# wuer5/OMGSR

Hardware: AMD Instinct MI355X
Metric: SR images/sec (higher is better)
Workload: dtype fp16; 1 GPU; OMGSR-S 256->1024, batch=4/GPU, accurate tier (fp32 stream, fp16 MFMA operands + split corrections), tiled VAE 256/64; global_batch=4, latent_tile=64, tile_overlap=32, world_size=1, parallelism=dp1, weights=seeded random, SD2.1-base shapes

## Files before the change

include/omgsr_hip.h:

```cpp
#ifndef OMGSR_HIP_H
#define OMGSR_HIP_H

#include <stdint.h>

#ifdef __cplusplus
extern "C" {
#endif

#define OMGSR_E_BADARG (-1)
#define OMGSR_E_SHAPE (-2)
#define OMGSR_E_ARCH (-3)

#define OMGSR_ACT_NONE 0
#define OMGSR_ACT_SILU 1
#define OMGSR_ACT_GELU_TANH 2
#define OMGSR_ACT_GEGLU 3

#define OMGSR_OUT_BF16 0
#define OMGSR_OUT_F32 1

#define OMGSR_LAYOUT_NHWC 0
#define OMGSR_LAYOUT_T 1

#define OMGSR_EL_16 0
// ... 108 lines not shown
                                 int32_t G, int32_t act, int32_t stat_rows, int32_t x_el, int32_t y_el, void* y2, int32_t y2_el,
                                 uint32_t* overflow_flag, void* stream);
typedef struct omgsr_gn_apply_group {
    const void* x;
    void* y;
    void* y2;
    int64_t HW;
    int32_t rows;
    int32_t reserved;
} omgsr_gn_apply_group;
int omgsr_groupnorm_apply_multi(const omgsr_gn_apply_group* groups, int32_t ngroups, const float* mean, const float* rstd,
                                const float* gamma, const float* beta, int32_t C, int32_t G, int32_t act, int32_t stat_rows,
                                int32_t x_el, int32_t y_el, int32_t y2_el, uint32_t* overflow_flag, void* stream);
int omgsr_groupnorm_apply_mxfp8(const void* x, void* codes, void* scales, const float* mean, const float* rstd, const float* gamma,
                                const float* beta, int32_t rows, int64_t HW, int32_t C, int32_t G, int32_t act, int32_t stat_rows,
                                int32_t x_el, void* stream);
int omgsr_groupnorm_apply_mxfp8_c64(const void* x, void* codes, void* scales, const float* mean, const float* rstd, const float* gamma,
                                    const float* beta, int32_t rows, int64_t HW, int32_t C, int32_t G, int32_t act, int32_t stat_rows,
                                    int32_t x_el, void* stream);
int omgsr_groupnorm_apply_mxfp8_multi(const omgsr_gn_apply_group* groups, int32_t ngroups, const float* mean, const float* rstd,
                                      const float* gamma, const float* beta, int32_t C, int32_t G, int32_t act, int32_t stat_rows,
                                      int32_t x_el, void* stream);
typedef struct omgsr_edge_group {
    const void* x;
    void* y;
    int32_t rows;
    int32_t H;
    int32_t W;
    int32_t reserved;
} omgsr_edge_group;
int omgsr_conv_out_gn(const omgsr_edge_group* groups, int32_t ngroups, const float* mean, const float* rstd, const float* gamma,
                      const float* beta, const float* weight, const float* bias, int32_t Cin, int32_t Cout, int32_t G, int32_t stat_rows,
                      void* stream);
int omgsr_groupnorm_finalize2(const float* partial_a, int32_t nslot_a, int32_t Ca, const float* partial_b, int32_t nslot_b, int32_t Cb,
                              float* mean, float* rstd, float* var_out, int32_t N, int32_t G, double count, float eps, void* stream);
int omgsr_groupnorm_apply2(const void* xa, const void* xb, int32_t Ca, void* y, const float* mean, const float* rstd, const float* gamma,
                           const float* beta, int32_t N, int64_t HW, int32_t C, int32_t G, int32_t act, int32_t y_el, void* y2, int32_t y2_el,
                           uint32_t* overflow_flag, void* stream);

int omgsr_layernorm(const void* x, void* y, const float* a, const float* b, int64_t rows, int32_t C,
                    float eps, int32_t x_el, int32_t y_el, void* stream);
int omgsr_quantize_mxfp8(const void* x, int32_t x_el, int64_t rows, int32_t K, int64_t x_ld, void* codes, void* scales, void* stream);
int omgsr_quantize_mxfp8_ld(const void* x, int32_t x_el, int64_t rows, int32_t K, int64_t x_ld, void* codes, void* scales, int64_t c_ld,
                            int64_t s_ld, void* stream);
int omgsr_layernorm_mxfp8(const void* x, const float* a, const float* b, int64_t rows, int32_t C, float eps, int32_t x_el, void* codes,
                          void* scales, int64_t c_ld, int64_t s_ld, void* stream);
int omgsr_to_operand(const float* x, void* y, int64_t rows, int32_t C, int32_t y_el, uint32_t* overflow_flag, void* stream);
int omgsr_transpose_split(const float* x, void* y, int32_t B, int32_t L, int32_t C, int64_t ld, void* stream);

typedef struct omgsr_attn_args {
    const void* q; const void* k; const void* vt; void* o;
    int32_t B, H, D, Lq, Lk;
    int64_t q_ld, k_ld, vt_ld, o_ld;
    int64_t q_bstride, k_bstride, vt_bstride, o_bstride;
    float scale;
    int32_t o_lo_off;
    int32_t o_mx;
    int32_t q_lo_off;
    int32_t k_lo_off;
    int32_t p_split;
    int32_t reserved1;
    int64_t vt_lo_off;
    int32_t qkv_el;
    int32_t qkv_reserved;
    const uint8_t* q_scale;
    const uint8_t* k_scale;
// ... 67 lines not shown
```

omgsr_amd/_lib.py:

```python
from __future__ import annotations

import ctypes as C
import os

import torch

from .build import lib_path

ABI_VERSION = 22


class OmgsrError(RuntimeError):
    pass


class IgemmArgs(C.Structure):
    _fields_ = [
        ("in_", C.c_void_p), ("weight", C.c_void_p), ("bias", C.c_void_p), ("gate", C.c_void_p),
        ("residual", C.c_void_p), ("out", C.c_void_p),
        ("N", C.c_int32), ("H", C.c_int32), ("W", C.c_int32), ("Cin", C.c_int32),
        ("Cout", C.c_int32), ("Cout_pad", C.c_int32), ("K_pad", C.c_int32),
        ("R", C.c_int32), ("S", C.c_int32), ("stride", C.c_int32), ("pad_top", C.c_int32),
        ("pad_left", C.c_int32), ("upsample", C.c_int32),
        ("Ho", C.c_int32), ("Wo", C.c_int32),
        ("act", C.c_int32), ("out_dtype", C.c_int32), ("out_layout", C.c_int32),
        ("t_rows", C.c_int32), ("t_ld", C.c_int32), ("out_ld", C.c_int32),
        ("batch", C.c_int32),
        ("in_bstride", C.c_int64), ("w_bstride", C.c_int64), ("out_bstride", C.c_int64),
        ("alpha", C.c_float), ("weight_cm", C.c_void_p), ("workspace", C.c_void_p),
        ("gn_partial", C.c_void_p), ("gn_groups", C.c_int32), ("gn_entries", C.c_int32),
        ("res_el", C.c_int32), ("in_split", C.c_int32), ("sample_rows", C.c_int64), ("out_lo_off", C.c_int32),
        ("in_ld", C.c_int32), ("w_split", C.c_int32), ("weight_ph", C.c_void_p), ("mx_chunks16", C.c_int32), ("mx_scale_w1", C.c_int32), ("mx_scale_a1", C.c_int32),
        ("mx_scale_w2", C.c_int32), ("mx_scale_a2", C.c_int32), ("out_mx", C.c_int32), ("group_tiles", C.c_int32), ("overflow_flag", C.c_void_p),
        ("gn_scale_shift", C.c_void_p), ("gn_nimg", C.c_int32), ("gn_act", C.c_int32), ("in_el", C.c_int32), ("mx_fmt", C.c_int32),
        ("mxf8", C.c_int32), ("mxf8_reserved", C.c_int32), ("in_scale", C.c_void_p), ("w_scale", C.c_void_p),
    ]


GN_MAX_GROUPS = 8


class GnMergeArgs(C.Structure):
    _fields_ = [("partial", C.c_void_p * GN_MAX_GROUPS), ("count", C.c_double * GN_MAX_GROUPS),
                ("weight", C.c_float * GN_MAX_GROUPS), ("tiles", C.c_int32 * GN_MAX_GROUPS),
                ("nslot", C.c_int32 * GN_MAX_GROUPS), ("entries", C.c_int32 * GN_MAX_GROUPS), ("ngroups", C.c_int32)]


class GnApplyGroup(C.Structure):
    _fields_ = [("x", C.c_void_p), ("y", C.c_void_p), ("y2", C.c_void_p), ("HW", C.c_int64), ("rows", C.c_int32), ("reserved", C.c_int32)]


class EdgeGroup(C.Structure):
    _fields_ = [("x", C.c_void_p), ("y", C.c_void_p), ("rows", C.c_int32), ("H", C.c_int32), ("W", C.c_int32), ("reserved", C.c_int32)]


class AttnArgs(C.Structure):
    _fields_ = [
        ("q", C.c_void_p), ("k", C.c_void_p), ("vt", C.c_void_p), ("o", C.c_void_p),
        ("B", C.c_int32), ("H", C.c_int32), ("D", C.c_int32), ("Lq", C.c_int32), ("Lk", C.c_int32),
        ("q_ld", C.c_int64), ("k_ld", C.c_int64), ("vt_ld", C.c_int64), ("o_ld", C.c_int64),
        ("q_bstride", C.c_int64), ("k_bstride", C.c_int64), ("vt_bstride", C.c_int64), ("o_bstride", C.c_int64),
        ("scale", C.c_float), ("o_lo_off", C.c_int32), ("o_mx", C.c_int32), ("q_lo_off", C.c_int32), ("k_lo_off", C.c_int32), ("p_split", C.c_int32),
        ("reserved1", C.c_int32), ("vt_lo_off", C.c_int64),
        ("qkv_el", C.c_int32), ("qkv_reserved", C.c_int32), ("q_scale", C.c_void_p), ("k_scale", C.c_void_p), ("vt_scale", C.c_void_p),
        ("q_sld", C.c_int64), ("k_sld", C.c_int64), ("vt_sld", C.c_int64), ("q_sbstride", C.c_int64), ("k_sbstride", C.c_int64),
        ("vt_sbstride", C.c_int64),
    ]


class TimingEntry(C.Structure):
    _fields_ = [("kind", C.c_int32), ("ms", C.c_float), ("flops", C.c_double), ("bytes", C.c_double),
                ("m", C.c_int64), ("n", C.c_int64), ("k", C.c_int64), ("variant", C.c_int32), ("stage", C.c_int32)]


_P, _I, _L, _F = C.c_void_p, C.c_int32, C.c_int64, C.c_float

SIGNATURES = {
    "omgsr_abi_version": (C.c_int, []),
    "omgsr_check_device": (C.c_int, []),
    "omgsr_set_compute_dtype": (C.c_int, [C.c_int]),
    "omgsr_get_compute_dtype": (C.c_int, []),
    "omgsr_error_string": (C.c_char_p, [C.c_int]),
    "omgsr_igemm": (C.c_int, [C.POINTER(IgemmArgs), _P]),
    "omgsr_igemm_out_mxfp8": (C.c_int, [C.POINTER(IgemmArgs), _P, _L, _P]),
    "omgsr_igemm_mxfp8_multi_ok": (C.c_int32, [C.POINTER(IgemmArgs), _I]),
    "omgsr_igemm_mxfp8_multi": (C.c_int, [C.POINTER(IgemmArgs), _I, _P]),
    "omgsr_igemm_multi_plan": (C.c_int, [C.POINTER(IgemmArgs), _I]),
    "omgsr_igemm_multi": (C.c_int, [C.POINTER(IgemmArgs), _I, _P]),
    "omgsr_set_batch_invariant": (C.c_int, [C.c_int]),
    "omgsr_set_attention_defer_max": (C.c_int, [C.c_float]),
    "omgsr_igemm_workspace_bytes": (C.c_int64, [C.POINTER(IgemmArgs)]),
    "omgsr_igemm_gn_slots": (C.c_int32, [C.POINTER(IgemmArgs)]),
    "omgsr_igemm_gn_entries": (C.c_int32, [C.POINTER(IgemmArgs)]),
    "omgsr_igemm_gn_fusable": (C.c_int32, [C.POINTER(IgemmArgs)]),
    "omgsr_igemm_out_mx6_ok": (C.c_int32, [C.POINTER(IgemmArgs)]),
    "omgsr_conv_mxfp8_ok": (C.c_int32, [C.POINTER(IgemmArgs)]),
    "omgsr_conv_mxfp8": (C.c_int, [C.POINTER(IgemmArgs), _P]),
    "omgsr_conv_mxfp8_multi_ok": (C.c_int32, [C.POINTER(IgemmArgs), _I]),
    "omgsr_conv_mxfp8_multi": (C.c_int, [C.POINTER(IgemmArgs), _I, _P]),
    "omgsr_conv_mxfp8_up_ok": (C.c_int32, [C.POINTER(IgemmArgs)]),
    "omgsr_conv_mxfp8_up": (C.c_int, [C.POINTER(IgemmArgs), _P]),
    "omgsr_conv_mxfp8_up_multi_ok": (C.c_int32, [C.POINTER(IgemmArgs), _I]),
    "omgsr_conv_mxfp8_up_multi": (C.c_int, [C.POINTER(IgemmArgs), _I, _P]),
    "omgsr_conv_mxfp8_deep_ok": (C.c_int32, [C.POINTER(IgemmArgs)]),
    "omgsr_conv_mxfp8_deep": (C.c_int, [C.POINTER(IgemmArgs), _P]),
    "omgsr_groupnorm_apply_mxfp8": (C.c_int, [_P, _P, _P, _P, _P, _P, _P, _I, _L, _I, _I, _I, _I, _I, _P]),
    "omgsr_groupnorm_apply_mxfp8_c64": (C.c_int, [_P, _P, _P, _P, _P, _P, _P, _I, _L, _I, _I, _I, _I, _I, _P]),
    "omgsr_groupnorm_apply_mxfp8_multi": (C.c_int, [C.POINTER(GnApplyGroup), _I, _P, _P, _P, _P, _I, _I, _I, _I, _I, _P]),
    "omgsr_groupnorm_scale_shift": (C.c_int, [_P, _P, _P, _P, _P, _I, _I, _I, _P]),
    "omgsr_groupnorm_finalize": (C.c_int, [_P, _P, _P, _P, _I, _I, _I, _I, C.c_double, _F, _P]),
    "omgsr_groupnorm_partial": (C.c_int, [_P, _P, _I, _L, _I, _I, _I, _P]),
    "omgsr_groupnorm_finalize_merged": (C.c_int, [C.POINTER(GnMergeArgs), _P, _P, _P, _I, _I, _F, _P]),
    "omgsr_groupnorm_apply_shared": (C.c_int, [_P, _P, _P, _P, _P, _P, _I, _L, _I, _I, _I, _I, _I, _I, _P, _I, _P, _P]),
    "omgsr_groupnorm_apply_multi": (C.c_int, [C.POINTER(GnApplyGroup), _I, _P, _P, _P, _P, _I, _I, _I, _I, _I, _I, _I, _P, _P]),
    "omgsr_conv_out_gn": (C.c_int, [C.POINTER(EdgeGroup), _I, _P, _P, _P, _P, _P, _P, _I, _I, _I, _I, _P]),
    "omgsr_groupnorm_finalize2": (C.c_int, [_P, _I, _I, _P, _I, _I, _P, _P, _P, _I, _I, C.c_double, _F, _P]),
    "omgsr_groupnorm_apply2": (C.c_int, [_P, _P, _I, _P, _P, _P, _P, _P, _I, _L, _I, _I, _I, _I, _P, _I, _P, _P]),
    "omgsr_image_to_model_input": (C.c_int, [_P, _P, _I, _I, _I, _I, _P]),
    "omgsr_colorfix_workspace_bytes": (C.c_int64, [_I, _I, _I, _I]),
    "omgsr_colorfix": (C.c_int, [_P, _I, _P, _P, _P, _I, _I, _I, _I, _I, _P]),
    "omgsr_groupnorm_nchunk": (C.c_int, [_L]),
    "omgsr_groupnorm_stats": (C.c_int, [_P, _P, _P, _P, _P, _I, _L, _I, _I, _F, _I, _P]),
    "omgsr_groupnorm_apply": (C.c_int, [_P, _P, _P, _P, _P, _P, _I, _L, _I, _I, _I, _I, _I, _P, _I, _P, _P]),
    "omgsr_layernorm": (C.c_int, [_P, _P, _P, _P, _L, _I, _F, _I, _I, _P]),
    "omgsr_resize_nearest_exact_nhwc": (C.c_int, [_P, _P, _I, _I, _I, _I, _I, _I, _F, _F, _I, _P]),
    "omgsr_transpose_split": (C.c_int, [_P, _P, _I, _I, _I, _L, _P]),
    "omgsr_to_operand": (C.c_int, [_P, _P, _L, _I, _I, _P, _P]),
    "omgsr_quantize_mxfp8": (C.c_int, [_P, _I, _L, _I, _L, _P, _P, _P]),
    "omgsr_quantize_mxfp8_ld": (C.c_int, [_P, _I, _L, _I, _L, _P, _P, _L, _L, _P]),
    "omgsr_layernorm_mxfp8": (C.c_int, [_P, _P, _P, _L, _I, _F, _I, _P, _P, _L, _L, _P]),
    "omgsr_attention": (C.c_int, [C.POINTER(AttnArgs), _P]),
    "omgsr_softmax_rows": (C.c_int, [_P, _P, _L, _I, _I, _P]),
    "omgsr_softmax_rows_split": (C.c_int, [_P, _P, _L, _I, _I, _P]),
    "omgsr_rmsnorm_rope": (C.c_int, [_P, _P, _P, _I, _P, _P, _I, _I, _I, _I, _L, _I, _I, _F, _P]),
    "omgsr_rmsnorm_rope_mxfp8": (C.c_int, [_P, _P, _P, _I, _P, _P, _I, _I, _I, _I, _L, _I, _I, _F, _P, _P, _L, _L, _P]),
    "omgsr_nchw_to_nhwc": (C.c_int, [_P, _P, _I, _I, _I, _I, _I, _I, _I, _P]),
    "omgsr_nhwc_to_nchw": (C.c_int, [_P, _P, _I, _I, _I, _I, _I, _I, _I, _F, _F, _I, _P]),
    "omgsr_copy_channels": (C.c_int, [_P, _P, _L, _I, _I, _I, _I, _I, _P]),
    "omgsr_vae_sample": (C.c_int, [_P, _P, _P, _L, _I, _I, _F, _F, _I, _P]),
    "omgsr_axpby": (C.c_int, [_P, _P, _P, _L, _F, _F, _F, _F, _I, _I, _P]),
    "omgsr_linear_f32": (C.c_int, [_P, _P, _P, _P, _I, _I, _I, _I, _P]),
    "omgsr_tile_accumulate": (C.c_int, [_P, _P, _P, _I, _I, _I, _I, _I, _I, _I, _I, _I, _I, _P]),
    "omgsr_tile_normalise": (C.c_int, [_P, _P, _P, _I, _L, _I, _I, _I, _P]),
    "omgsr_crop_nhwc": (C.c_int, [_P, _P, _I, _I, _I, _I, _I, _I, _I, _I, _I, _P]),
    "omgsr_paste_nhwc": (C.c_int, [_P, _P] + [_I] * 13 + [_P]),
    "omgsr_flux_pack": (C.c_int, [_P, _P, _I, _I, _I, _I, _I, _I, _I, _P]),
    "omgsr_resample_u8": (C.c_int, [_P, _P, _P, _P, _I, _I, _I, _I, _I, _I, _P]),
    "omgsr_timing_enable": (C.c_int, [C.c_int]),
# ... 37 lines not shown
```

omgsr_amd/build.py:

```python
from __future__ import annotations

import hashlib
import os
import shutil
import subprocess
import sys

HERE = os.path.dirname(os.path.abspath(__file__))
CSRC = os.path.join(HERE, "csrc")
LIBDIR = os.path.join(HERE, "lib")
LIBNAME = "libomgsr_hip.so"
SOURCES = ["igemm.hip", "igemm_dma.hip", "igemm_p8.hip", "igemm_gmx.hip", "igemm_halo.hip", "igemm_halo_f16.hip", "igemm_halo_multi.hip", "igemm_halo_mx.hip", "igemm_halo_mx6.hip", "igemm_halo_mx6_flat.hip", "igemm_halo_out6.hip", "igemm_halo_flat.hip", "igemm_halo_gn.hip", "attention.hip", "norm.hip", "elementwise.hip", "colorfix.hip", "preprocess.hip", "mfma_peak.hip", "gemm_mxfp8.hip", "gemm_mxfp8_out8.hip", "gemm_mxfp8_multi.hip", "attention_mxfp8.hip", "attention_d512.hip", "conv_mxfp8.hip", "conv_mxfp8_up.hip", "conv_mxfp8_deep.hip", "conv_edge.hip"]
ARCH = "gfx950"


def lib_path() -> str:
    return os.path.join(LIBDIR, LIBNAME)


def _source_digest() -> str:
    h = hashlib.sha256()
    names = sorted(os.listdir(CSRC)) + [os.path.join("..", "..", "include", "omgsr_hip.h")]
    for n in names:
        p = os.path.join(CSRC, n)
        if os.path.isfile(p):
            h.update(n.encode())
            with open(p, "rb") as f:
                h.update(f.read())
    return h.hexdigest()


def build_library(force: bool = False, verbose: bool = False) -> str:
    hipcc = shutil.which("hipcc") or "/opt/rocm/bin/hipcc"
    os.makedirs(LIBDIR, exist_ok=True)
    out = lib_path()
    stamp = out + ".sha256"
    defs = ["-DOMGSR_BUILD_ABLATIONS"] if os.environ.get("OMGSR_BUILD_ABLATIONS", "0") == "1" else []
    defs += os.environ.get("OMGSR_EXTRA_DEFS", "").split()
    digest = _source_digest() + "".join(defs)
    if not force and os.path.isfile(out) and os.path.isfile(stamp) and open(stamp).read().strip() == digest:
        return out
    if not os.path.exists(hipcc):
        raise RuntimeError("hipcc not found: cannot build libomgsr_hip.so")
    from concurrent.futures import ThreadPoolExecutor

# ... 117 lines not shown
```

omgsr_amd/diffusers_api/autoencoder_kl.py:

```python
from __future__ import annotations

import os
from types import SimpleNamespace
from typing import Optional

import torch
import torch.nn as nn

from .. import ops
from ..nn import Conv2d, GroupNorm, Linear, norm_silu_conv
from .modeling_utils import ConfigDict, ModelMixin

SD21_VAE_CONFIG = dict(in_channels=3, out_channels=3, block_out_channels=[128, 256, 512, 512], layers_per_block=2,
                       latent_channels=4, norm_num_groups=32, scaling_factor=0.18215, shift_factor=None,
                       use_quant_conv=True, use_post_quant_conv=True, act_fn="silu", sample_size=768)
FLUX_VAE_CONFIG = dict(in_channels=3, out_channels=3, block_out_channels=[128, 256, 512, 512], layers_per_block=2,
                       latent_channels=16, norm_num_groups=32, scaling_factor=0.3611, shift_factor=0.1159,
                       use_quant_conv=False, use_post_quant_conv=False, act_fn="silu", sample_size=1024)


class ResnetBlock2D(nn.Module):
    def __init__(self, in_channels: int, out_channels: int, temb_channels: Optional[int], groups: int, eps: float):
        super().__init__()
        self.in_channels, self.out_channels = in_channels, out_channels
        self.norm1 = GroupNorm(groups, in_channels, eps=eps)
        self.conv1 = Conv2d(in_channels, out_channels, 3, padding=1)
        self.time_emb_proj = Linear(temb_channels, out_channels) if temb_channels else None
        self.norm2 = GroupNorm(groups, out_channels, eps=eps)
        self.conv2 = Conv2d(out_channels, out_channels, 3, padding=1)
        self.use_in_shortcut = in_channels != out_channels
        self.conv_shortcut = Conv2d(in_channels, out_channels, 1) if self.use_in_shortcut else None
        self.nonlinearity = nn.SiLU()

    def nhwc(self, x, conv1_bias=None, out_for=None):
        if isinstance(x, tuple):
            h, xc = self.norm1.nhwc_pair(x[0], x[1], ops.ACT_SILU, split=self.conv1.in_split(), also_cast=self.conv_shortcut.in_split())
            h = self.conv1.nhwc(h, bias_override=conv1_bias, gn_groups=self.norm2.num_groups)
        elif self.conv_shortcut is not None and x.dtype == torch.float32:
            h, xc = self.norm1.nhwc(x, ops.ACT_SILU, split=self.conv1.in_split(), also_cast=self.conv_shortcut.in_split())
            h = self.conv1.nhwc(h, bias_override=conv1_bias, gn_groups=self.norm2.num_groups)
        else:
            xc = x
            h = self.conv1.nhwc(x, gn=self.norm1.spec(x, ops.ACT_SILU), bias_override=conv1_bias, gn_groups=self.norm2.num_groups)
        g2 = self.norm2.spec(h, ops.ACT_SILU)
        sc = self.conv_shortcut.nhwc(xc, pad=0) if self.conv_shortcut is not None else x
        if out_for is not None:
            return self.conv2.nhwc(h, gn=g2, residual=sc, out_dtype=ops.OUT_BF16, out_split=out_for.in_split())
        return self.conv2.nhwc(h, gn=g2, residual=sc, gn_groups=self.norm1.num_groups)

    def forward(self, x, temb=None):
        if temb is not None or self.time_emb_proj is not None:
            raise NotImplementedError("ResnetBlock2D.forward: the UNet folds the time embedding at fixed t* (UNet2DConditionModel.nhwc)")
        return _nchw_call(self.nhwc, x, self.out_channels)


class Downsample2D(nn.Module):
    def __init__(self, channels: int, padding: int):
        super().__init__()
        self.padding = padding
        self.conv = Conv2d(channels, channels, 3, stride=2, padding=padding)

    def nhwc(self, x, gn_groups: int = 0):
        pad = (0, 1, 0, 1) if self.padding == 0 else self.padding
        return self.conv.nhwc(x, pad=pad, gn_groups=gn_groups)

    def forward(self, x):
        return _nchw_call(self.nhwc, x, self.conv.out_channels)


class Upsample2D(nn.Module):
    def __init__(self, channels: int):
        super().__init__()
        self.conv = Conv2d(channels, channels, 3, padding=1)
        self.conv.phase_upsample = True

    def nhwc(self, x, gn_groups: int = 0):
        return self.conv.nhwc(x, upsample=True, gn_groups=gn_groups)

# ... 325 lines not shown
```

omgsr_amd/nn.py:

```python
from __future__ import annotations

import dataclasses
from typing import Optional

import torch
import torch.nn as nn

from . import ops


def _key(*tensors) -> tuple:
    return ops.mode_key() + tuple((t.data_ptr(), t._version, str(t.device), t.dtype, tuple(t.shape)) if torch.is_tensor(t) else t for t in tensors)


_CACHE_EPOCH = 0


def cache_epoch() -> int:
    return _CACHE_EPOCH


def bump_cache_epoch() -> None:
    global _CACHE_EPOCH
    _CACHE_EPOCH += 1
# ... 111 lines not shown
        k = _key(self.weight, self.bias, "mxfp8-conv-deep")
        if getattr(self, "_pk8d_key", None) != k:
            bump_cache_epoch()
            _log_rebuild(self._drop_packed_mxfp8_deep)
            self._pk8d = ops.pack_conv_weight_mxfp8(self.weight, self.bias, cin_multiple=64)
            self._pk8d_key = k
        return self._pk8d

    def _drop_packed_mxfp8_deep(self) -> None:
        self._pk8d, self._pk8d_key = None, None
        bump_cache_epoch()

    def edge_out(self, x: torch.Tensor, norm: "GroupNorm") -> bool:
        return (self.groups == 1 and self.dilation == (1, 1) and self.stride[0] == self.stride[1] and self.padding[0] == self.padding[1]
                and x.shape[-1] == self.in_channels
                and ops.edge_conv_out_ok(x.dtype, self.weight.shape, self.stride[0], self.padding[0], norm.num_groups))

    def packed_edge_out(self) -> "ops.EdgeWeight":
        k = _key(self.weight, self.bias, "edge-out")
        if getattr(self, "_pke_key", None) != k:
            bump_cache_epoch()
            _log_rebuild(self._drop_packed_edge_out)
            self._pke = ops.pack_edge_out_weight(self.weight, self.bias)
            self._pke_key = k
        return self._pke

    def _drop_packed_edge_out(self) -> None:
        self._pke, self._pke_key = None, None
        bump_cache_epoch()

    def nhwc_edge_out_multi(self, xs, norm: "GroupNorm", mean: torch.Tensor, rstd: torch.Tensor):
        g, b = norm._affine()
        return ops.conv_out_gn_multi(list(xs), self.packed_edge_out(), mean, rstd, g, b, norm.num_groups)

    def packed(self) -> ops.PackedWeight:
        sp, wsp, ph = self.in_split(), self.in_wsplit(), self.phase_upsample
        return self._packed(lambda: ops.pack_conv_weight(self.weight, self.bias, cout_multiple=8, split=sp, w_split=wsp, upsample_phases=ph),
                            self.weight, self.bias, sp, wsp, ph)

    def nhwc(self, x, *, pad=None, upsample=False, act=ops.ACT_NONE, residual=None, bias_override=None, stride=None, gn_groups=0,
             out_dtype=ops.OUT_STREAM, out_split=1, gn=None):
        pw = self.packed()
        if bias_override is not None:
            pw = dataclasses.replace(pw, bias=bias_override)
        p = self.padding[0] if pad is None else pad
        if out_dtype == ops.OUT_STREAM and self.out_inner16 and ops.precise():
            out_dtype = ops.OUT_BF16
        fp8_pack = self.packed_mxfp8 if (self.fp8 and gn is not None and bias_override is None) else None
        fp8_up_pack = self.packed_mxfp8_up if (self.fp8_up and upsample and gn is None and bias_override is None) else None
        fp8_deep_pack = None
        if self.fp8_deep and gn is not None and self.in_channels % 64 == 0:
            fp8_deep_pack = self.packed_mxfp8_deep if bias_override is None else \
                (lambda: dataclasses.replace(self.packed_mxfp8_deep(), bias=bias_override))
        return ops.conv2d(x, pw, stride=stride or self.stride[0], pad=p, upsample=upsample, act=act, residual=residual,
                          gn_groups=gn_groups, out_dtype=out_dtype, out_split=out_split, gn=gn, fp8_pack=fp8_pack, fp8_up_pack=fp8_up_pack,
                          fp8_deep_pack=fp8_deep_pack)

    def nhwc_multi(self, xs, *, pad=None, upsample=False, act=ops.ACT_NONE, residuals=None, stride=None, gn_groups=0,
                   out_dtype=ops.OUT_STREAM, out_split=1, gn=None, fp8=False):
        pw = self.packed()
        p = self.padding[0] if pad is None else pad
        if out_dtype == ops.OUT_STREAM and self.out_inner16 and ops.precise():
            out_dtype = ops.OUT_BF16
        fp8_pack = self.packed_mxfp8 if (fp8 and self.fp8 and gn is not None) else None
        fp8_up_pack = self.packed_mxfp8_up if (fp8 and self.fp8_up and upsample and gn is None) else None
        return ops.conv2d_multi(list(xs), pw, stride=stride or self.stride[0], pad=p, upsample=upsample, act=act, residuals=residuals,
# ... 27 lines not shown
    def _affine(self):
        return self._packed(lambda: (self.weight.detach().float().contiguous(), self.bias.detach().float().contiguous()),
                            self.weight, self.bias)

    def nhwc(self, x, act=ops.ACT_NONE, split=1, also_cast=0):
        g, b = self._affine()
        return ops.group_norm(x, g, b, self.num_groups, self.eps, act, split=split, also_cast=also_cast)

    def nhwc_pair(self, a, b, act=ops.ACT_NONE, split=1, also_cast=0):
        g, bt = self._affine()
        return ops.group_norm_pair(a, b, g, bt, self.num_groups, self.eps, act, split=split, also_cast=also_cast)

    def stats(self, x):
        return ops.group_norm_stats(x, self.num_groups, self.eps)

    def spec(self, x, act=ops.ACT_NONE) -> "ops.GnSpec":
        mean, rstd, _ = self.stats(x)
        return self.spec_stats(mean, rstd, act)

    def spec_stats(self, mean, rstd, act=ops.ACT_NONE) -> "ops.GnSpec":
        g, b = self._affine()
        return ops.GnSpec(mean, rstd, g, b, self.num_groups, act)

    def apply_stats(self, x, mean, rstd, act=ops.ACT_NONE, split=1, also_cast=0):
        g, b = self._affine()
        if mean.shape[0] != x.shape[0]:
            return ops.group_norm_apply_shared(x, mean, rstd, g, b, self.num_groups, act, split=split, also_cast=also_cast)
        return ops.group_norm_apply(x, mean, rstd, g, b, self.num_groups, act, split=split, also_cast=also_cast)

    def apply_stats_multi(self, xs, mean, rstd, act=ops.ACT_NONE, split=1, also_cast=0):
        g, b = self._affine()
        return ops.group_norm_apply_multi(xs, mean, rstd, g, b, self.num_groups, act, split=split, also_cast=also_cast)

    def forward(self, x):
        shp = x.shape
        x4 = x.reshape(shp[0], shp[1], -1, 1) if x.dim() == 3 else x
        y = self.nhwc(ops.nchw_to_nhwc(x4.contiguous()))
        return ops.nhwc_to_nchw(y, dtype=ops.io_dtype(x)).to(x.dtype).reshape(shp)


def norm_silu_conv(norm: GroupNorm, conv: Conv2d, h: torch.Tensor) -> torch.Tensor:
    if conv.edge_out(h, norm):
        mean, rstd, _ = norm.stats(h)
        return conv.nhwc_edge_out_multi([h], norm, mean, rstd)[0]
    return conv.nhwc(h, gn=norm.spec(h, ops.ACT_SILU))


class LayerNorm(nn.LayerNorm, _Packed):
    def _affine(self):
        if not self.elementwise_affine:
            return None, None
        return self._packed(lambda: (self.weight.detach().float().contiguous(), self.bias.detach().float().contiguous()),
                            self.weight, self.bias)

    def nhwc(self, x, a=None, b=None, split=1):
        if a is None and b is None:
            a, b = self._affine()
        return ops.layer_norm(x, a, b, self.eps, split=split)

    def forward(self, x):
        return self.nhwc(x.to(ops.stream_dtype()).contiguous()).to(x.dtype)


class RMSNormWeight(nn.Module):

    def __init__(self, dim: int, eps: float):
# ... 7 lines not shown
```

omgsr_amd/ops.py:

```python
from __future__ import annotations

import ctypes as C
import os
from contextlib import contextmanager
from dataclasses import dataclass
from typing import NamedTuple, Optional

import torch

from . import _lib
from ._lib import AttnArgs, IgemmArgs, check

ACT_NONE, ACT_SILU, ACT_GELU_TANH, ACT_GEGLU = 0, 1, 2, 3
OUT_STREAM, OUT_BF16, OUT_F32 = -1, 0, 1
LAYOUT_NHWC, LAYOUT_T = 0, 1
EL_16, EL_F32, EL_SPLIT, EL_MX, EL_MX6, EL_MXFP8 = 0, 1, 2, 3, 4, 5
MX_LO_SHIFT = 11


def _el_of_split(split: int) -> int:
    return {1: EL_16, 2: EL_SPLIT, 3: EL_MX, 4: EL_MX6}[split]


_ACT = torch.bfloat16
# ... 1470 lines not shown
    w[..., :cout] = weight.detach().to(device=dev, dtype=torch.float32).reshape(cout, cin // 4, 4, 3, 3).permute(1, 3, 4, 2, 0)
    b = torch.zeros((cp,), device=dev, dtype=torch.float32)
    if bias is not None:
        b[:cout] = bias.detach().to(device=dev, dtype=torch.float32)
    return EdgeWeight(w.contiguous(), b, cin, cout)


def conv_out_gn_multi(xs, ew: EdgeWeight, mean: torch.Tensor, rstd: torch.Tensor, gamma: torch.Tensor, beta: torch.Tensor, groups: int,
                      one_launch: bool = True):
    if not 0 < len(xs) <= _lib.GN_MAX_GROUPS:
        raise ValueError(f"1 ... {_lib.GN_MAX_GROUPS} tile shape groups")
    for x in xs:
        if _req(x, torch.float32, "x").dim() != 4 or x.shape[-1] != ew.cin:
            raise ValueError(f"conv_out_gn: x must be [rows, H, W, {ew.cin}]")
    outs = [torch.empty((*x.shape[:-1], 8), device=x.device, dtype=torch.float32) for x in xs]
    desc = (_lib.EdgeGroup * len(xs))()
    for k, x in enumerate(xs):
        desc[k].x, desc[k].y = x.data_ptr(), outs[k].data_ptr()
        desc[k].rows, desc[k].H, desc[k].W = x.shape[0], x.shape[1], x.shape[2]
    fn = _lib.load().omgsr_conv_out_gn
    for first, count in ([(0, len(xs))] if one_launch else [(k, 1) for k in range(len(xs))]):
        check(fn(C.byref(desc[first]), count, _req(mean, torch.float32, "mean").data_ptr(), _req(rstd, torch.float32, "rstd").data_ptr(),
                 _req(gamma, torch.float32, "gamma").data_ptr(), _req(beta, torch.float32, "beta").data_ptr(), ew.w.data_ptr(),
                 ew.bias.data_ptr(), ew.cin, ew.cout, groups, mean.shape[0], _stream()), "omgsr_conv_out_gn")
    return outs


def conv_out_gn(x: torch.Tensor, ew: EdgeWeight, mean: torch.Tensor, rstd: torch.Tensor, gamma: torch.Tensor, beta: torch.Tensor,
                groups: int) -> torch.Tensor:
    return conv_out_gn_multi([x], ew, mean, rstd, gamma, beta, groups)[0]



def layer_norm(x: torch.Tensor, a: Optional[torch.Tensor], b: Optional[torch.Tensor], eps: float, split: int = 1) -> torch.Tensor:
    xel = _el(x, "x")
    Cc = x.shape[-1]
    rows = x.numel() // Cc
    y = _operand_like(x, split)
    check(_lib.load().omgsr_layernorm(x.data_ptr(), y.data_ptr(), _ptr(a), _ptr(b), rows, Cc, eps, xel, _el_of_split(split), _stream()),
          "omgsr_layernorm")
    return y


def layer_norm_mxfp8(x: torch.Tensor, a: Optional[torch.Tensor], b: Optional[torch.Tensor], eps: float, out: Optional[Mxfp8] = None) -> Mxfp8:
    if x.dtype != torch.bfloat16 or _ACT != torch.bfloat16 or _PRECISE:
        raise ValueError("layer_norm_mxfp8: a bf16 stream tensor under the bf16 compute type (the fp8 tier)")
    _req(x, torch.bfloat16, "x")
    Cc = x.shape[-1]
    if Cc % 128 or Cc > 4096:
        raise ValueError(f"layer_norm_mxfp8: C = {Cc} must be a multiple of 128, at most 4096")
    if out is None:
        out = _mxfp8_like(x)
    elif out.codes.shape != x.shape or out.scales.shape != (*x.shape[:-1], Cc // 32) or not (out.codes.is_contiguous() and out.scales.is_contiguous()):
        raise ValueError("layer_norm_mxfp8: `out` does not match x")
    check(_lib.load().omgsr_layernorm_mxfp8(x.data_ptr(), _ptr(a), _ptr(b), x.numel() // Cc, Cc, eps, EL_16, out.codes.data_ptr(), out.scales.data_ptr(),
                                            Cc, Cc // 32, _stream()), "omgsr_layernorm_mxfp8")
    return out



def attention(q: torch.Tensor, k: torch.Tensor, vt: torch.Tensor, heads: int, head_dim: int, scale: float,
              *, q_col: int = 0, k_col: int = 0, Lk: Optional[int] = None, out: Optional[torch.Tensor] = None,
              o_col: int = 0, out_split: int = 1, o_lo_col: Optional[int] = None, q_lo_col: Optional[int] = None,
              k_lo_col: Optional[int] = None, p_split: bool = True) -> torch.Tensor:
    mx = [isinstance(x, Mxfp8) for x in (q, k, vt)]
    if any(mx):
# ... 293 lines not shown
```

omgsr_amd/pipelines/vaehook.py:

```python
from __future__ import annotations

import math
from typing import Dict, List, Tuple

import torch

from .. import ops


def get_best_tile_size(lowerbound: int, upperbound: int) -> int:
    divider = 32
    while divider >= 2:
        rem = lowerbound % divider
        if rem == 0:
            return lowerbound
        cand = lowerbound - rem + divider
        if cand <= upperbound:
            return cand
        divider //= 2
    return lowerbound


def split_tiles(h: int, w: int, tile_size: int, pad: int, is_decoder: bool) -> Tuple[List[List[int]], List[List[int]]]:
    nh = max(math.ceil((h - 2 * pad) / tile_size), 1)
# ... 72 lines not shown
        return self.vae_tile_forward(x)

    def _run(self, seq, groups: Dict[tuple, torch.Tensor], counts: Dict[tuple, int], N: int, fixed=None, record=None):
        res: Dict[tuple, list] = {k: [] for k in groups}
        gi = 0
        pending = None
        edge = None
        for op in seq:
            kind = op[0]
            if kind == "gn":
                norm, act = op[1], op[2]
                G = norm.num_groups
                if fixed is not None:
                    mean, var = fixed[gi]
                    rstd = torch.rsqrt(var + 1e-6)
                else:
                    keys = list(groups)
                    mean, rstd, var = ops.group_norm_stats_merged([groups[k] for k in keys], [counts[k] for k in keys], N, G, 1e-6)
                if record is not None:
                    record.append((mean, var))
                gi += 1
                first = next(iter(groups.values()))
                is_conv3 = getattr(op[3], "kernel_size", None) == (3, 3)
                if op[3] is self.net.conv_out and act == ops.ACT_SILU and op[4] is None and op[3].edge_out(first, norm):
                    edge = (norm, mean, rstd)
                    continue
                if is_conv3 and first.dtype != torch.float32:
                    pending = norm.spec_stats(mean, rstd, act)
                    if op[4] is not None:
                        for k in groups:
                            res[k].append(op[4].nhwc(groups[k], pad=0))
                    continue
                keys = list(groups)
                if op[4] is not None:
                    outs = norm.apply_stats_multi([groups[k] for k in keys], mean, rstd, act, split=op[3].in_split(), also_cast=op[4].in_split())
                    for k, (y, xc) in zip(keys, outs):
                        groups[k] = y
                        res[k].append(op[4].nhwc(xc, pad=0))
                else:
                    for k, y in zip(keys, norm.apply_stats_multi([groups[k] for k in keys], mean, rstd, act, split=op[3].in_split())):
                        groups[k] = y
            elif kind == "conv":
                keys = list(groups)
                if edge is not None:
                    outs = op[1].nhwc_edge_out_multi([groups[k] for k in keys], *edge)
                    edge = None
                else:
                    outs = op[1].nhwc_multi([groups[k] for k in keys], gn=pending, fp8=self.fp8_convs, **op[2])
                for k, y in zip(keys, outs):
                    groups[k] = y
                pending = None
            elif kind == "res_push":
                for k in groups:
                    res[k].append(op[1](groups[k]) if op[1] is not None else groups[k])
            elif kind == "conv_res":
                keys = list(groups)
                xs, rs = [groups[k] for k in keys], [res[k].pop() for k in keys]
                if op[3] is not None:
                    outs = op[1].nhwc_multi(xs, residuals=rs, out_dtype=ops.OUT_BF16, out_split=op[3].in_split(), gn=pending, fp8=self.fp8_convs)
                else:
                    outs = op[1].nhwc_multi(xs, residuals=rs, gn_groups=op[2], gn=pending, fp8=self.fp8_convs)
                pending = None
                for k, y in zip(keys, outs):
                    groups[k] = y
            elif kind == "attn_res":
                for k in groups:
                    groups[k] = op[1].attend(groups[k], residual=res[k].pop())
# ... 43 lines not shown
```

Before: 21.67 images/s.

## Fuse GroupNorm apply with 1x1 shortcut conv in VAE resnet blocks

Adds a HIP kernel that reads the fp32 input once and writes two outputs: the normalized, SiLU-activated operand for conv1, and the 1x1 shortcut convolution of the raw input. The shortcut uses fp16 hi/lo split MFMA with three products to keep fp32-level accuracy. This replaces a separate cast pass and a separate shortcut conv launch, cutting a global-memory round trip and one kernel per resnet block in the tiled VAE. The cost is extra epilogue LDS traffic, more register pressure, and a fixed tile shape that may use the GPU less well than the dedicated conv kernel.

New measurement: 22.02 images/s (median of 6 runs). 1.6% higher.

```diff
diff --git a/include/omgsr_hip.h b/include/omgsr_hip.h
--- a/include/omgsr_hip.h
+++ b/include/omgsr_hip.h
@@ -164,6 +164,18 @@
 int omgsr_conv_out_gn(const omgsr_edge_group* groups, int32_t ngroups, const float* mean, const float* rstd, const float* gamma,
                       const float* beta, const float* weight, const float* bias, int32_t Cin, int32_t Cout, int32_t G, int32_t stat_rows,
                       void* stream);
+typedef struct omgsr_gn_shortcut_group {
+    const void* x;
+    void* y;
+    void* sc;
+    int64_t HW;
+    int32_t rows;
+    int32_t reserved;
+} omgsr_gn_shortcut_group;
+int32_t omgsr_groupnorm_shortcut_ok(int32_t C, int32_t N, int32_t G, int32_t y_el);
+int omgsr_groupnorm_shortcut(const omgsr_gn_shortcut_group* groups, int32_t ngroups, const float* mean, const float* rstd,
+                             const float* gamma, const float* beta, const void* weight, const float* bias, int32_t C, int32_t N,
+                             int32_t G, int32_t act, int32_t stat_rows, int32_t y_el, uint32_t* overflow_flag, void* stream);
 int omgsr_groupnorm_finalize2(const float* partial_a, int32_t nslot_a, int32_t Ca, const float* partial_b, int32_t nslot_b, int32_t Cb,
                               float* mean, float* rstd, float* var_out, int32_t N, int32_t G, double count, float eps, void* stream);
 int omgsr_groupnorm_apply2(const void* xa, const void* xb, int32_t Ca, void* y, const float* mean, const float* rstd, const float* gamma,
diff --git a/omgsr_amd/_lib.py b/omgsr_amd/_lib.py
--- a/omgsr_amd/_lib.py
+++ b/omgsr_amd/_lib.py
@@ -52,6 +52,10 @@
 
 class EdgeGroup(C.Structure):
     _fields_ = [("x", C.c_void_p), ("y", C.c_void_p), ("rows", C.c_int32), ("H", C.c_int32), ("W", C.c_int32), ("reserved", C.c_int32)]
+
+
+class GnShortcutGroup(C.Structure):
+    _fields_ = [("x", C.c_void_p), ("y", C.c_void_p), ("sc", C.c_void_p), ("HW", C.c_int64), ("rows", C.c_int32), ("reserved", C.c_int32)]
 
 
 class AttnArgs(C.Structure):
@@ -114,6 +118,8 @@
     "omgsr_groupnorm_apply_shared": (C.c_int, [_P, _P, _P, _P, _P, _P, _I, _L, _I, _I, _I, _I, _I, _I, _P, _I, _P, _P]),
     "omgsr_groupnorm_apply_multi": (C.c_int, [C.POINTER(GnApplyGroup), _I, _P, _P, _P, _P, _I, _I, _I, _I, _I, _I, _I, _P, _P]),
     "omgsr_conv_out_gn": (C.c_int, [C.POINTER(EdgeGroup), _I, _P, _P, _P, _P, _P, _P, _I, _I, _I, _I, _P]),
+    "omgsr_groupnorm_shortcut_ok": (C.c_int32, [_I, _I, _I, _I]),
+    "omgsr_groupnorm_shortcut": (C.c_int, [C.POINTER(GnShortcutGroup), _I, _P, _P, _P, _P, _P, _P, _I, _I, _I, _I, _I, _I, _P, _P]),
     "omgsr_groupnorm_finalize2": (C.c_int, [_P, _I, _I, _P, _I, _I, _P, _P, _P, _I, _I, C.c_double, _F, _P]),
     "omgsr_groupnorm_apply2": (C.c_int, [_P, _P, _I, _P, _P, _P, _P, _P, _I, _L, _I, _I, _I, _I, _P, _I, _P, _P]),
     "omgsr_image_to_model_input": (C.c_int, [_P, _P, _I, _I, _I, _I, _P]),
diff --git a/omgsr_amd/build.py b/omgsr_amd/build.py
--- a/omgsr_amd/build.py
+++ b/omgsr_amd/build.py
@@ -10,7 +10,7 @@
 CSRC = os.path.join(HERE, "csrc")
 LIBDIR = os.path.join(HERE, "lib")
 LIBNAME = "libomgsr_hip.so"
-SOURCES = ["igemm.hip", "igemm_dma.hip", "igemm_p8.hip", "igemm_gmx.hip", "igemm_halo.hip", "igemm_halo_f16.hip", "igemm_halo_multi.hip", "igemm_halo_mx.hip", "igemm_halo_mx6.hip", "igemm_halo_mx6_flat.hip", "igemm_halo_out6.hip", "igemm_halo_flat.hip", "igemm_halo_gn.hip", "attention.hip", "norm.hip", "elementwise.hip", "colorfix.hip", "preprocess.hip", "mfma_peak.hip", "gemm_mxfp8.hip", "gemm_mxfp8_out8.hip", "gemm_mxfp8_multi.hip", "attention_mxfp8.hip", "attention_d512.hip", "conv_mxfp8.hip", "conv_mxfp8_up.hip", "conv_mxfp8_deep.hip", "conv_edge.hip"]
+SOURCES = ["igemm.hip", "igemm_dma.hip", "igemm_p8.hip", "igemm_gmx.hip", "igemm_halo.hip", "igemm_halo_f16.hip", "igemm_halo_multi.hip", "igemm_halo_mx.hip", "igemm_halo_mx6.hip", "igemm_halo_mx6_flat.hip", "igemm_halo_out6.hip", "igemm_halo_flat.hip", "igemm_halo_gn.hip", "attention.hip", "norm.hip", "elementwise.hip", "colorfix.hip", "preprocess.hip", "mfma_peak.hip", "gemm_mxfp8.hip", "gemm_mxfp8_out8.hip", "gemm_mxfp8_multi.hip", "attention_mxfp8.hip", "attention_d512.hip", "conv_mxfp8.hip", "conv_mxfp8_up.hip", "conv_mxfp8_deep.hip", "conv_edge.hip", "norm_shortcut.hip"]
 ARCH = "gfx950"
 
 
diff --git a/omgsr_amd/csrc/norm_shortcut.hip b/omgsr_amd/csrc/norm_shortcut.hip
--- /dev/null
+++ b/omgsr_amd/csrc/norm_shortcut.hip
@@ -0,0 +1,217 @@
+#include "common.hip.h"
+#include "timing.hip.h"
+#include "../../include/omgsr_hip.h"
+
+namespace {
+
+constexpr int GS_CK = 64;
+constexpr int GS_ROW = 9;
+constexpr int GS_MAXC = 512;
+constexpr int GS_EP_LD = 36;
+
+struct GnShortcutTable {
+    const float* x[OMGSR_GN_MAX_GROUPS];
+    void* y[OMGSR_GN_MAX_GROUPS];
+    float* sc[OMGSR_GN_MAX_GROUPS];
+    int HW[OMGSR_GN_MAX_GROUPS];
+    int tiles[OMGSR_GN_MAX_GROUPS];
+    int start[OMGSR_GN_MAX_GROUPS + 1];
+    int count;
+};
+
+template <int PT, int NTW, int YEL>
+__global__ __launch_bounds__(256, 2) void gn_shortcut_kernel(const GnShortcutTable m, const float* __restrict__ mean, const float* __restrict__ rstd,
+                                                              const float* __restrict__ gamma, const float* __restrict__ beta,
+                                                              const u32x4_t* __restrict__ wpk, const float* __restrict__ bias,
+                                                              const int C, const int G, const int act, const int stat_rows,
+                                                              unsigned* __restrict__ ovf) {
+    using T = f16_t;
+    constexpr int P = 32 * PT, NT = 4 * NTW, N = 32 * NT;
+    static_assert(2 * P * GS_ROW * 16 >= 4 * 32 * GS_EP_LD * 4, "the epilogue's four transpose tiles reuse the operand tile");
+    __shared__ __attribute__((aligned(16))) u32x4_t tile[2 * P * GS_ROW];
+    __shared__ __attribute__((aligned(16))) float tab[2 * GS_MAXC];
+    const int t = threadIdx.x, lane = t & 63;
+    const int wave = __builtin_amdgcn_readfirstlane(t >> 6);
+    int s = 0;
+    while (s + 1 < m.count && (int)blockIdx.x >= m.start[s + 1]) ++s;
+    const int local = (int)blockIdx.x - m.start[s];
+    const int n = local / m.tiles[s];
+    const int HW = m.HW[s];
+    const int p0 = (local - n * m.tiles[s]) * P;
+    const float* __restrict__ x = m.x[s];
+    void* __restrict__ y = m.y[s];
+    float* __restrict__ scout = m.sc[s];
+
+    float* sc = tab;
+    float* sh = tab + C;
+    const int ns = n % stat_rows;
+    const int cpg = C / G;
+    for (int c = t; c < C; c += 256) {
+        const int g = c / cpg;
+        const float r = rstd[ns * G + g], mu = mean[ns * G + g];
+        const float a = r * (gamma ? gamma[c] : 1.0f);
+        sc[c] = a;
+        sh[c] = (beta ? beta[c] : 0.0f) - mu * a;
+    }
+    __syncthreads();
+    auto transform = [&](float (&f)[8], const int cc) {
+        const f32x4_t* sa = reinterpret_cast<const f32x4_t*>(sc + cc * 8);
+        const f32x4_t* ha = reinterpret_cast<const f32x4_t*>(sh + cc * 8);
+        const f32x4_t sa0 = sa[0], sa1 = sa[1], ha0 = ha[0], ha1 = ha[1];
+#pragma unroll
+        for (int e = 0; e < 8; ++e) {
+            const float v = f[e] * (e < 4 ? sa0[e & 3] : sa1[e & 3]) + (e < 4 ? ha0[e & 3] : ha1[e & 3]);
+            f[e] = (act == OMGSR_ACT_SILU) ? silu_f(v) : v;
+        }
+    };
+
+    const int oct = t & 7, prow = t >> 3;
+    const int64_t pix0 = (int64_t)n * HW + p0;
+    float raw[PT][8];
+    auto fetch = [&](const int chunk) {
+#pragma unroll
+        for (int i = 0; i < PT; ++i) {
+            if (p0 + prow + 32 * i < HW) load8<T, true>(x, (pix0 + prow + 32 * i) * C + chunk * GS_CK + oct * 8, raw[i]);
+            else {
+#pragma unroll
+                for (int e = 0; e < 8; ++e) raw[i][e] = 0.0f;
+            }
+        }
+    };
+
+    f32x16_t acc[PT][NTW];
+#pragma unroll
+    for (int i = 0; i < PT; ++i)
+#pragma unroll
+        for (int j = 0; j < NTW; ++j)
+#pragma unroll
+            for (int r = 0; r < 16; ++r) acc[i][j][r] = 0.0f;
+    float amax = 0.0f;
+
+    u32x4_t* thi = tile;
+    u32x4_t* tlo = tile + P * GS_ROW;
+    const int arow = (lane & 31) * GS_ROW + (lane >> 5);
+    const int nchunk = C / GS_CK;
+    fetch(0);
+    for (int chunk = 0; chunk < nchunk; ++chunk) {
+#pragma unroll
+        for (int i = 0; i < PT; ++i) {
+            u32x4_t hi, lo;
+            split8<T>(raw[i], hi, lo);
+            thi[(prow + 32 * i) * GS_ROW + oct] = hi;
+            tlo[(prow + 32 * i) * GS_ROW + oct] = lo;
+#pragma unroll
+            for (int e = 0; e < 8; ++e) amax = fmaxf(amax, fabsf(raw[i][e]));
+        }
+#pragma unroll
+        for (int i = 0; i < PT; ++i) {
+            const bool valid = p0 + prow + 32 * i < HW;
+            const int64_t pix = valid ? pix0 + prow + 32 * i : pix0;
+            const int cc8 = chunk * 8 + oct;
+            float f[8];
+#pragma unroll
+            for (int e = 0; e < 8; ++e) f[e] = raw[i][e];
+            transform(f, cc8);
+            if constexpr (YEL == OMGSR_EL_MX6) store8_mx6<T>(y, pix * 4 * C, C, cc8 * 8, f, valid);
+            else if (valid) store8<T, 0>(y, pix * C + cc8 * 8, C, f);
+        }
+        __syncthreads();
+        if (chunk + 1 < nchunk) fetch(chunk + 1);
+        const u32x4_t* wc = wpk + ((int64_t)chunk * 4 * NT + wave * NTW) * 128 + lane;
+#pragma unroll
+        for (int ks = 0; ks < 4; ++ks) {
+            u32x4_t bh[NTW], bl[NTW];
+#pragma unroll
+            for (int j = 0; j < NTW; ++j) {
+                bh[j] = wc[(ks * NT + j) * 128];
+                bl[j] = wc[(ks * NT + j) * 128 + 64];
+            }
+#pragma unroll
+            for (int i = 0; i < PT; ++i) {
+                const u32x4_t ah = thi[i * 32 * GS_ROW + arow + 2 * ks], al = tlo[i * 32 * GS_ROW + arow + 2 * ks];
+                const f16x8_t ahv = *reinterpret_cast<const f16x8_t*>(&ah), alv = *reinterpret_cast<const f16x8_t*>(&al);
+#pragma unroll
+                for (int j = 0; j < NTW; ++j) {
+                    const f16x8_t bhv = *reinterpret_cast<const f16x8_t*>(&bh[j]), blv = *reinterpret_cast<const f16x8_t*>(&bl[j]);
+                    acc[i][j] = mfma32(ahv, bhv, acc[i][j]);
+                    acc[i][j] = mfma32(alv, bhv, acc[i][j]);
+                    acc[i][j] = mfma32(ahv, blv, acc[i][j]);
+                }
+            }
+        }
+        __syncthreads();
+    }
+    if (ovf && __any(amax > 65504.0f) && lane == 0) atomicOr(ovf, 1u);
+
+    float* ep = reinterpret_cast<float*>(tile) + wave * (32 * GS_EP_LD);
+#pragma unroll
+    for (int i = 0; i < PT; ++i) {
+#pragma unroll
+        for (int j = 0; j < NTW; ++j) {
+            if (i + j) __syncthreads();
+#pragma unroll
+            for (int r = 0; r < 16; ++r) ep[cfrag_row(lane, r) * GS_EP_LD + (lane & 31)] = acc[i][j][r];
+            __syncthreads();
+            const int col = (wave * NTW + j) * 32 + (lane & 7) * 4;
+            const f32x4_t b = bias ? *reinterpret_cast<const f32x4_t*>(bias + col) : (f32x4_t){0.0f, 0.0f, 0.0f, 0.0f};
+#pragma unroll
+            for (int q = 0; q < 4; ++q) {
+                const int row = q * 8 + (lane >> 3);
+                const f32x4_t v = *reinterpret_cast<const f32x4_t*>(ep + row * GS_EP_LD + (lane & 7) * 4);
+                if (p0 + i * 32 + row < HW) *reinterpret_cast<f32x4_t*>(scout + (pix0 + i * 32 + row) * N + col) = v + b;
+            }
+        }
+    }
+}
+
+template <int PT, int NTW>
+int launch_el(const int y_el, const dim3 grid, hipStream_t st, const GnShortcutTable& m, const float* mean, const float* rstd, const float* gamma,
+              const float* beta, const void* w, const float* bias, int C, int G, int act, int stat_rows, unsigned* ovf) {
+    const u32x4_t* wp = (const u32x4_t*)w;
+    if (y_el == OMGSR_EL_MX6) hipLaunchKernelGGL((gn_shortcut_kernel<PT, NTW, OMGSR_EL_MX6>), grid, dim3(256), 0, st, m, mean, rstd, gamma, beta, wp, bias, C, G, act, stat_rows, ovf);
+    else hipLaunchKernelGGL((gn_shortcut_kernel<PT, NTW, OMGSR_EL_16>), grid, dim3(256), 0, st, m, mean, rstd, gamma, beta, wp, bias, C, G, act, stat_rows, ovf);
+    return (int)hipGetLastError();
+}
+
+int tile_pixels(const int N) { return N == 512 ? 64 : N == 256 ? 96 : 128; }
+
+}
+
+extern "C" int32_t omgsr_groupnorm_shortcut_ok(int32_t C, int32_t N, int32_t G, int32_t y_el) {
+    const bool ch = (C == 128 || C == 256 || C == 512) && (N == 128 || N == 256 || N == 512);
+    return ch && G > 0 && C % G == 0 && (y_el == OMGSR_EL_16 || y_el == OMGSR_EL_MX6) && omgsr::compute_dtype() == 1;
+}
+
+extern "C" int omgsr_groupnorm_shortcut(const omgsr_gn_shortcut_group* groups, int32_t ngroups, const float* mean, const float* rstd,
+                                        const float* gamma, const float* beta, const void* weight, const float* bias, int32_t C, int32_t N,
+                                        int32_t G, int32_t act, int32_t stat_rows, int32_t y_el, uint32_t* overflow_flag, void* stream) {
+    if (!groups || ngroups <= 0 || ngroups > OMGSR_GN_MAX_GROUPS || !mean || !rstd || !weight || C <= 0 || N <= 0 || G <= 0 || stat_rows <= 0)
+        return OMGSR_E_BADARG;
+    if (!omgsr_groupnorm_shortcut_ok(C, N, G, y_el) || (act != OMGSR_ACT_NONE && act != OMGSR_ACT_SILU)) return OMGSR_E_SHAPE;
+    const int P = tile_pixels(N);
+    GnShortcutTable m;
+    memset(&m, 0, sizeof(m));
+    int64_t blocks = 0;
+    double pixels = 0.0;
+    for (int k = 0; k < ngroups; ++k) {
+        const omgsr_gn_shortcut_group& g = groups[k];
+        if (!g.x || !g.y || !g.sc || g.rows <= 0 || g.HW <= 0) return OMGSR_E_BADARG;
+        if (g.HW >= (1ll << 31) - P) return OMGSR_E_SHAPE;
+        m.x[k] = (const float*)g.x; m.y[k] = g.y; m.sc[k] = (float*)g.sc; m.HW[k] = (int)g.HW;
+        m.tiles[k] = (int)((g.HW + P - 1) / P);
+        m.start[k] = (int)blocks;
+        blocks += (int64_t)g.rows * m.tiles[k];
+        if (blocks >= (1ll << 31)) return OMGSR_E_SHAPE;
+        pixels += (double)g.rows * (double)g.HW;
+    }
+    m.start[ngroups] = (int)blocks;
+    m.count = ngroups;
+    hipStream_t st = (hipStream_t)stream;
+    omgsr::TimingScope ts(OMGSR_TK_IGEMM, 2.0 * pixels * N * C, pixels * (4.0 * C + (y_el == OMGSR_EL_MX6 ? 4.0 : 2.0) * C + 4.0 * N) + 4.0 * C * N, st,
+                          (long long)pixels, N, C);
+    if (ts.active) ts.rec.variant = 29;
+    const dim3 grid((unsigned)blocks);
+    if (N == 128) return launch_el<4, 1>(y_el, grid, st, m, mean, rstd, gamma, beta, weight, bias, C, G, act, stat_rows, overflow_flag);
+    if (N == 256) return launch_el<3, 2>(y_el, grid, st, m, mean, rstd, gamma, beta, weight, bias, C, G, act, stat_rows, overflow_flag);
+    return launch_el<2, 4>(y_el, grid, st, m, mean, rstd, gamma, beta, weight, bias, C, G, act, stat_rows, overflow_flag);
+}
diff --git a/omgsr_amd/diffusers_api/autoencoder_kl.py b/omgsr_amd/diffusers_api/autoencoder_kl.py
--- a/omgsr_amd/diffusers_api/autoencoder_kl.py
+++ b/omgsr_amd/diffusers_api/autoencoder_kl.py
@@ -36,6 +36,10 @@
         if isinstance(x, tuple):
             h, xc = self.norm1.nhwc_pair(x[0], x[1], ops.ACT_SILU, split=self.conv1.in_split(), also_cast=self.conv_shortcut.in_split())
             h = self.conv1.nhwc(h, bias_override=conv1_bias, gn_groups=self.norm2.num_groups)
+        elif self.conv_shortcut is not None and x.dtype == torch.float32 and self.conv_shortcut.gn_shortcut(x, self.norm1, self.conv1.in_split()):
+            h, sc = self.norm1.nhwc_shortcut(x, self.conv_shortcut, ops.ACT_SILU, split=self.conv1.in_split())
+            h = self.conv1.nhwc(h, bias_override=conv1_bias, gn_groups=self.norm2.num_groups)
+            xc = None
         elif self.conv_shortcut is not None and x.dtype == torch.float32:
             h, xc = self.norm1.nhwc(x, ops.ACT_SILU, split=self.conv1.in_split(), also_cast=self.conv_shortcut.in_split())
             h = self.conv1.nhwc(h, bias_override=conv1_bias, gn_groups=self.norm2.num_groups)
@@ -43,7 +47,8 @@
             xc = x
             h = self.conv1.nhwc(x, gn=self.norm1.spec(x, ops.ACT_SILU), bias_override=conv1_bias, gn_groups=self.norm2.num_groups)
         g2 = self.norm2.spec(h, ops.ACT_SILU)
-        sc = self.conv_shortcut.nhwc(xc, pad=0) if self.conv_shortcut is not None else x
+        if xc is not None:
+            sc = self.conv_shortcut.nhwc(xc, pad=0) if self.conv_shortcut is not None else x
         if out_for is not None:
             return self.conv2.nhwc(h, gn=g2, residual=sc, out_dtype=ops.OUT_BF16, out_split=out_for.in_split())
         return self.conv2.nhwc(h, gn=g2, residual=sc, gn_groups=self.norm1.num_groups)
diff --git a/omgsr_amd/nn.py b/omgsr_amd/nn.py
--- a/omgsr_amd/nn.py
+++ b/omgsr_amd/nn.py
@@ -167,6 +167,24 @@
     def nhwc_edge_out_multi(self, xs, norm: "GroupNorm", mean: torch.Tensor, rstd: torch.Tensor):
         g, b = norm._affine()
         return ops.conv_out_gn_multi(list(xs), self.packed_edge_out(), mean, rstd, g, b, norm.num_groups)
+
+    def gn_shortcut(self, x: torch.Tensor, norm: "GroupNorm", split: int) -> bool:
+        return (self.groups == 1 and self.dilation == (1, 1) and self.stride[0] == self.stride[1] and self.padding[0] == self.padding[1]
+                and x.shape[-1] == self.in_channels == norm.num_channels and not self.out_inner16
+                and ops.gn_shortcut_ok(x.dtype, self.weight.shape, self.stride[0], self.padding[0], norm.num_groups, split))
+
+    def packed_gn_shortcut(self) -> "ops.ShortcutWeight":
+        k = _key(self.weight, self.bias, "gn-shortcut")
+        if getattr(self, "_pks_key", None) != k:
+            bump_cache_epoch()
+            _log_rebuild(self._drop_packed_gn_shortcut)
+            self._pks = ops.pack_gn_shortcut_weight(self.weight, self.bias)
+            self._pks_key = k
+        return self._pks
+
+    def _drop_packed_gn_shortcut(self) -> None:
+        self._pks, self._pks_key = None, None
+        bump_cache_epoch()
 
     def packed(self) -> ops.PackedWeight:
         sp, wsp, ph = self.in_split(), self.in_wsplit(), self.phase_upsample
@@ -260,6 +278,15 @@
         g, b = self._affine()
         return ops.group_norm_apply_multi(xs, mean, rstd, g, b, self.num_groups, act, split=split, also_cast=also_cast)
 
+    def nhwc_shortcut(self, x, shortcut: "Conv2d", act=ops.ACT_NONE, split=1):
+        g, b = self._affine()
+        mean, rstd, _ = ops.group_norm_stats(x, self.num_groups, self.eps)
+        return ops.group_norm_shortcut(x, shortcut.packed_gn_shortcut(), mean, rstd, g, b, self.num_groups, act, split)
+
+    def apply_stats_shortcut_multi(self, xs, mean, rstd, shortcut: "Conv2d", act=ops.ACT_NONE, split=1):
+        g, b = self._affine()
+        return ops.group_norm_shortcut_multi(list(xs), shortcut.packed_gn_shortcut(), mean, rstd, g, b, self.num_groups, act, split)
+
     def forward(self, x):
         shp = x.shape
         x4 = x.reshape(shp[0], shp[1], -1, 1) if x.dim() == 3 else x
diff --git a/omgsr_amd/ops.py b/omgsr_amd/ops.py
--- a/omgsr_amd/ops.py
+++ b/omgsr_amd/ops.py
@@ -1526,6 +1526,79 @@
 
 
 
+GN_SHORTCUT_CHANNELS = (128, 256, 512)
+GN_SHORTCUT_SPLITS = (1, 4)
+
+
+@dataclass
+class ShortcutWeight:
+    w: torch.Tensor
+    bias: torch.Tensor
+    cin: int
+    cout: int
+
+
+def gn_shortcut_enabled() -> bool:
+    return os.environ.get("OMGSR_GN_SHORTCUT_FUSED", "1") != "0"
+
+
+def gn_shortcut_ok(stream: torch.dtype, weight_shape, stride: int, padding: int, groups: int, split: int) -> bool:
+    if len(weight_shape) != 4:
+        return False
+    cout, cin, kh, kw = (int(v) for v in weight_shape)
+    return (gn_shortcut_enabled() and _PRECISE and _ACT == torch.float16 and stream == torch.float32 and (kh, kw) == (1, 1) and stride == 1
+            and padding == 0 and cin in GN_SHORTCUT_CHANNELS and cout in GN_SHORTCUT_CHANNELS and groups > 0 and cin % groups == 0
+            and split in GN_SHORTCUT_SPLITS)
+
+
+def pack_gn_shortcut_weight(weight: torch.Tensor, bias: Optional[torch.Tensor], device=None) -> ShortcutWeight:
+    cout, cin = int(weight.shape[0]), int(weight.shape[1])
+    if tuple(weight.shape[2:]) != (1, 1) or cin % 64 or cout % 32:
+        raise ValueError("pack_gn_shortcut_weight: a 1x1 kernel, Cin % 64 == 0, Cout % 32 == 0")
+    dev = device or weight.device
+    w = _note_weight_range(weight.detach().to(device=dev, dtype=torch.float32).reshape(cout, cin))
+    hi = w.to(torch.float16)
+    lo = (w - hi.float()).to(torch.float16)
+
+    def frag(m):
+        return m.reshape(cout // 32, 32, cin // 64, 4, 2, 8).permute(2, 3, 0, 4, 1, 5)
+
+    pk = torch.stack((frag(hi), frag(lo)), dim=3).contiguous().reshape(cin // 64, 4, cout // 32, 2, 64, 8)
+    b = torch.zeros((cout,), device=dev, dtype=torch.float32)
+    if bias is not None:
+        b.copy_(bias.detach().to(device=dev, dtype=torch.float32))
+    return ShortcutWeight(pk, b, cin, cout)
+
+
+def group_norm_shortcut_multi(xs, sw: ShortcutWeight, mean: torch.Tensor, rstd: torch.Tensor, gamma, beta, groups: int, act: int = ACT_NONE,
+                              split: int = 1, one_launch: bool = True):
+    if not 0 < len(xs) <= _lib.GN_MAX_GROUPS:
+        raise ValueError(f"1 ... {_lib.GN_MAX_GROUPS} tile shape groups")
+    if split not in GN_SHORTCUT_SPLITS:
+        raise ValueError("group_norm_shortcut: y is a plain (split 1) or MX6 (split 4) operand")
+    for x in xs:
+        if _req(x, torch.float32, "x").shape[-1] != sw.cin:
+            raise ValueError(f"group_norm_shortcut: x must be [rows, ..., {sw.cin}]")
+    ys = [_operand_like(x, split) for x in xs]
+    scs = [torch.empty((*x.shape[:-1], sw.cout), device=x.device, dtype=torch.float32) for x in xs]
+    desc = (_lib.GnShortcutGroup * len(xs))()
+    for k, x in enumerate(xs):
+        desc[k].x, desc[k].y, desc[k].sc = x.data_ptr(), ys[k].data_ptr(), scs[k].data_ptr()
+        desc[k].rows, desc[k].HW = x.shape[0], x.numel() // (x.shape[0] * sw.cin)
+    fn = _lib.load().omgsr_groupnorm_shortcut
+    for first, count in ([(0, len(xs))] if one_launch else [(k, 1) for k in range(len(xs))]):
+        check(fn(C.byref(desc[first]), count, _req(mean, torch.float32, "mean").data_ptr(), _req(rstd, torch.float32, "rstd").data_ptr(),
+                 _ptr(gamma), _ptr(beta), sw.w.data_ptr(), sw.bias.data_ptr(), sw.cin, sw.cout, groups, act, mean.shape[0],
+                 _el_of_split(split), _ovf(xs[0].device), _stream()), "omgsr_groupnorm_shortcut")
+    return list(zip(ys, scs))
+
+
+def group_norm_shortcut(x: torch.Tensor, sw: ShortcutWeight, mean: torch.Tensor, rstd: torch.Tensor, gamma, beta, groups: int,
+                        act: int = ACT_NONE, split: int = 1):
+    return group_norm_shortcut_multi([x], sw, mean, rstd, gamma, beta, groups, act, split)[0]
+
+
+
 def layer_norm(x: torch.Tensor, a: Optional[torch.Tensor], b: Optional[torch.Tensor], eps: float, split: int = 1) -> torch.Tensor:
     xel = _el(x, "x")
     Cc = x.shape[-1]
diff --git a/omgsr_amd/pipelines/vaehook.py b/omgsr_amd/pipelines/vaehook.py
--- a/omgsr_amd/pipelines/vaehook.py
+++ b/omgsr_amd/pipelines/vaehook.py
@@ -128,7 +128,12 @@
                             res[k].append(op[4].nhwc(groups[k], pad=0))
                     continue
                 keys = list(groups)
-                if op[4] is not None:
+                if op[4] is not None and op[4].gn_shortcut(first, norm, op[3].in_split()):
+                    outs = norm.apply_stats_shortcut_multi([groups[k] for k in keys], mean, rstd, op[4], act, split=op[3].in_split())
+                    for k, (y, sc) in zip(keys, outs):
+                        groups[k] = y
+                        res[k].append(sc)
+                elif op[4] is not None:
                     outs = norm.apply_stats_multi([groups[k] for k in keys], mean, rstd, act, split=op[3].in_split(), also_cast=op[4].in_split())
                     for k, (y, xc) in zip(keys, outs):
                         groups[k] = y
```
